# lizaibeim/mmla-audio

Measured on AMD Instinct MI355X. Metric: audio clips/sec (MFCC→logits) at 1/2/4/8 MI355X; MFCC max-abs-err vs librosa, higher is better.
Workload: dtype f16x3+f32

## Files before the change

### mmla_audio_amd/csrc/context.cpp

```cpp
#include <algorithm>
#include <cstdarg>
#include <cstdio>
#include <cstdlib>

#include "internal.h"

using namespace mmla;

namespace mmla __attribute__((visibility("hidden"))) {

int fail(mmla_ctx* c, int code, const char* fmt, ...) {
  char buf[512];
  va_list ap;
  va_start(ap, fmt);
  vsnprintf(buf, sizeof(buf), fmt, ap);
  va_end(ap);
  if (c) c->err = buf;
  return code;
}

static hipEvent_t prof_event(mmla_ctx* c) {
  if (!c->prof_pool.empty()) {
    hipEvent_t e = c->prof_pool.back();
    c->prof_pool.pop_back();
// ... 134 lines not shown
  double held = 0;
  for (size_t i = 0; i < c->ws_size.size(); ++i)
    if (!slot_kept((int)i)) held += (double)c->ws_size[i];
  int64_t fit = (int64_t)(((double)fr + held) * 0.9 / (od ? kOdBytesPerClip : kSiBytesPerClip));
  fit = fit / kMinMicrobatch * kMinMicrobatch;
  return std::max(kMinMicrobatch, std::min(cap, fit));
}

}

struct EnvSwitch {
  const char* name;
  bool mmla_ctx::*no;
  int mmla_ctx::*num;
};
static const EnvSwitch kEnvSwitches[] = {
    {"MMLA_DEBUG_FAIL_ALLOC", nullptr, &mmla_ctx::debug_fail_allocs},
    {"MMLA_NO_SIU", &mmla_ctx::siu, nullptr},
    {"MMLA_NO_SIPU", &mmla_ctx::sipu, nullptr},
    {"MMLA_NO_SIFIN", &mmla_ctx::sifin, nullptr},
    {"MMLA_NO_SIPAIR", &mmla_ctx::sipair, nullptr},
    {"MMLA_NO_SICHAIN", &mmla_ctx::sichain, nullptr},
    {"MMLA_NO_LSTM_SPLIT", &mmla_ctx::lstm_split, nullptr},
    {"MMLA_LSTM_SPLIT_MAX", nullptr, &mmla_ctx::lstm_split_max},
    {"MMLA_DEBUG_LSTM_SPIN", nullptr, &mmla_ctx::lstm_spin},
    {"MMLA_DEBUG_TRACE_GUARD", nullptr, &mmla_ctx::debug_trace_guard},
    {"MMLA_NO_SIPAD", &mmla_ctx::si_pad_feat, nullptr},
    {"MMLA_NO_ODU", &mmla_ctx::odu, nullptr},
    {"MMLA_NO_ODW", &mmla_ctx::odw, nullptr},
    {"MMLA_NO_VADW", &mmla_ctx::vadw, nullptr},
    {"MMLA_VADW", nullptr, &mmla_ctx::vadw_all},
    {"MMLA_RB_TILE", &mmla_ctx::rbs, nullptr},
    {"MMLA_NO_RBS_W1L", &mmla_ctx::rbs_w1l, nullptr},
    {"MMLA_NO_RBS_TAILPAIR", &mmla_ctx::rbs_tailpair, nullptr},
    {"MMLA_NO_PIN_OUT", &mmla_ctx::pin_small, nullptr},
};

extern "C" {

int mmla_abi_version(void) { return MMLA_ABI_VERSION; }

int mmla_create(int device, mmla_ctx** out) {
  if (!out) return MMLA_E_INVALID;
  *out = nullptr;
  int ndev = 0;
  if (hipGetDeviceCount(&ndev) != hipSuccess || ndev == 0) return MMLA_E_HIP;
  if (device < 0 || device >= ndev) return MMLA_E_INVALID;
  if (hipSetDevice(device) != hipSuccess) return MMLA_E_HIP;
  mmla_ctx* c = new mmla_ctx();
  c->device = device;
  for (const EnvSwitch& s : kEnvSwitches)
    if (const char* v = std::getenv(s.name)) {
      if (s.no) c->*s.no = std::atoi(v) == 0;
      else c->*s.num = std::atoi(v);
    }
  if (hipStreamCreateWithFlags(&c->own_stream, hipStreamDefault) != hipSuccess) {
    delete c;
    return MMLA_E_HIP;
  }
  c->stream = c->own_stream;
  if (hipMalloc(&c->range_dev, RW_COUNT * sizeof(int)) != hipSuccess ||
      hipMemset(c->range_dev, 0, RW_COUNT * sizeof(int)) != hipSuccess ||
      hipHostMalloc(&c->range_host, 2 * sizeof(int), hipHostMallocDefault) != hipSuccess) {
    mmla_destroy(c);
    return MMLA_E_HIP;
  }
// ... 173 lines not shown
```

### mmla_audio_amd/csrc/internal.h

```cpp
#pragma once
#include <hip/hip_runtime.h>

#include <cstdint>
#include <cstring>
#include <string>
#include <vector>

#include "../../include/mmla.h"
#include "nr.h"
#include "od_fe.h"
#include "mix.h"
#include "si_fe.h"
#include "ssim.h"
#include "vad.h"

namespace mmla __attribute__((visibility("hidden"))) {

constexpr int OD_H = 128, OD_W = 151, OD_PIX = OD_H * OD_W;
constexpr int OD_IMG = OD_PIX * 3;
constexpr int SI_T = 256, SI_D = 39;
constexpr int SI_NEED_SAMPLES = 160 * 259 + 400;
constexpr int CH[9] = {32, 32, 32, 64, 64, 64, 128, 128, 128};
constexpr bool POOL[9] = {true, false, false, true, false, false, true, false, false};

// ... 66 lines not shown
  double prof_work[MMLA_NSTAGES] = {0};
  int64_t prof_n[MMLA_NSTAGES] = {0};
  int device = 0;
  hipStream_t stream = nullptr;
  hipStream_t own_stream = nullptr;
  std::string err;
  OdFeTables* od_tables = nullptr;
  SiFeTables* si_tables = nullptr;
  bool od_loaded = false, si_loaded = false;
  mmla::OdNet od;
  mmla::SiNet si;
  std::vector<void*> od_allocs, si_allocs;
  std::vector<void*> si_head_allocs;
  std::vector<void*> ws;
  std::vector<size_t> ws_size;
  std::vector<size_t> ws_guard;
  int64_t od_mb = 0, si_mb = 0;
  int64_t od_mb_cap = mmla::kOdMicrobatch, si_mb_cap = mmla::kSiMicrobatch;
  int debug_fail_allocs = 0;
  int debug_trace_guard = 0;
  int precision = MMLA_PREC_F16X3;
  bool siu = true;
  bool sipu = true;
  bool sifin = true;
  bool sipair = true;
  bool sichain = true;
  bool si_pad_feat = true;
  bool odu = true;
  bool odw = true;
  bool vadw = true;
  int vadw_all = 0;
  bool rbs = true;
  bool rbs_w1l = true;
  bool rbs_tailpair = true;
  bool lstm_split = true;
  int lstm_split_max = 128;
  int lstm_spin = 0;
  int* range_dev = nullptr;
  int* range_host = nullptr;
  bool pin_small = true;
  int* range_map = nullptr;
  int* range_map_dev = nullptr;
  char* pin_out = nullptr;
  char* pin_out_dev = nullptr;
  char* pin_in = nullptr;
  int64_t lstm_split_reruns = 0;
  int64_t range_reruns = 0;
  bool od_f32_only = false, si_f32_only = false;
  bool si_base_f16_bad = false;
  VadState* vad_state = nullptr;
  int64_t vad_streams = 0;
  int32_t* cap_state = nullptr;
  int cap_cur = 0;
  int64_t cap_streams = 0;
  int32_t cap_rate = 0, cap_channels = 0, cap_channel = 0, cap_ir = 0, cap_or = 0;
  NrTables* nr_tables = nullptr;
  float* nr_thresh = nullptr;
  int64_t nr_profiles = 0;
  bool nr_ready = false;
  int32_t nr_bank_sr = 0;
  double ns_time_constant_s = 2.0, ns_thresh_n_mult = 2.0, ns_sigmoid_slope = 10.0;
  int32_t ns_sr = 16000;
};

namespace mmla __attribute__((visibility("hidden"))) {

// ... 128 lines not shown
```

### mmla_audio_amd/csrc/net_runners.cpp

```cpp
#include <algorithm>

#include "conv.h"
#include "conv_h3.h"
#include "internal.h"
#include "nets.h"
#include "odu.h"
#include "resblk.h"
#include "siu.h"

using namespace mmla;

namespace {

ConvArgs conv_args(const ConvW& w, const float* x, float* y, int n, int h, int wd, int stride,
                   const BnW* bn, int pro, int epi, const float* res) {
  ConvArgs a{};
  a.x = x;
  a.wt = w.wt;
  a.bias = w.bias;
  a.scale = bn ? bn->scale : nullptr;
  a.shift = bn ? bn->shift : nullptr;
  a.res = res;
  a.y = y;
  a.n = n;
// ... 93 lines not shown
}

double lstm_flops(int64_t n, int T, int D) { return 2.0 * n * T * 2 * (256.0 + D) * 1024.0; }

hipError_t lstm_run(mmla_ctx* c, const Arith& ar, const LstmW& L, const float* seq, int64_t n, int T, float* out) {
  if (ar.h3() && L.wth[0] && ar.split &&
      n <= std::min(c->lstm_split_max, bilstm_h3_split_max_clips())) {
    void* ws = nullptr;
    if (ws_get(c, S_LSTM, bilstm_h3_split_ws_bytes(), &ws) != MMLA_OK) return hipErrorOutOfMemory;
    return bilstm_h3_split_launch(seq, (int)n, T, 128, L.wth[0], L.wtl[0], L.wth[1], L.wtl[1],
                                  L.bias[0], L.bias[1], out, ar.range, L.ws[0], L.ws[1], ws,
                                  ar.timeout, c->lstm_spin, c->stream);
  }
  if (ar.h3() && L.wth[0])
    return bilstm_h3_launch(seq, (int)n, T, 128, L.wth[0], L.wtl[0], L.wth[1], L.wtl[1], L.bias[0],
                            L.bias[1], out, ar.range, L.ws[0], L.ws[1], c->stream);
  return bilstm_launch(seq, (int)n, T, 128, L.wcat[0], L.wcat[1], L.bias[0], L.bias[1], out,
                       c->stream);
}


enum OdPath {
  OD_STRIPS,
  OD_TILES,
  OD_ODU,
  OD_PAIR
};
struct OdChoice {
  OdPath path;
  bool stem;
  int strips;
  bool w1_lds;
  bool tail_pair;
};

bool strips_ok(const ResUnitW& B, bool pool, int h, int w) {
  return B.ca.wh && B.cb.wh && (!pool || B.sc.wh) && B.ca.cin_pad == B.ca.cin && B.ca.cout_pad == 32 &&
         B.cb.cin_pad == 32 && B.cb.cout_pad == 32 && B.cb.kh == 4 && B.cb.kw == 1 &&
         (!pool || (B.sc.cin_pad == B.ca.cin && B.sc.cout_pad == 32)) &&
         rbs_supported(h, w, B.ca.cin, B.ca.cout, pool);
}

bool tiles_ok(const ResUnitW& B, bool pool) {
  return B.ca.fh && B.cb.fh && B.cb.kpad == 4 * B.cb.cin && (!pool || B.sc.fh) &&
         resblk_supported(B.ca.cin, B.ca.cout, pool);
}

bool odu_ok(const ResUnitW& B, bool pool, int h, int w) {
  return B.ca.wh && B.cb.wh && (!pool || B.sc.wh) && odu_supported(h, w, B.ca.cin, B.ca.cout, pool) &&
         B.ca.cin_pad == B.ca.cin && B.ca.cout_pad == B.ca.cout && B.cb.cin == B.ca.cout &&
         B.cb.cout == B.ca.cout && B.cb.cin_pad == B.cb.cin && B.cb.cout_pad == B.cb.cout &&
         B.cb.kh == 4 && B.cb.kw == 1 &&
         (!pool || (B.sc.cin == B.ca.cin && B.sc.cout == B.ca.cout && B.sc.cout_pad == B.sc.cout));
}

OdChoice od_choose(const mmla_ctx* c, const Arith& ar, const ResUnitW& B, int b, int h, int w, int stop) {
  OdChoice k{OD_PAIR, false, 1, false, false};
  if (!ar.h3()) return k;
  if (c->rbs && strips_ok(B, POOL[b], h, w)) {
    k.path = OD_STRIPS;
    k.w1_lds = c->rbs_w1l && !POOL[b];
    k.tail_pair = c->rbs_tailpair && POOL[b];
  } else if (tiles_ok(B, POOL[b])) {
    k.path = OD_TILES;
  } else if (c->odu && odu_ok(B, POOL[b], h, w)) {
    k.path = OD_ODU;
    k.strips = c->odw && odu_two_strips(h, w, B.ca.cin, B.ca.cout, POOL[b]) ? 2 : 1;
  }
  k.stem = b == 0 && stop != 0 && (k.path == OD_STRIPS || k.path == OD_TILES);
  return k;
}

ResBlkArgs resblk_args(const ResUnitW& B, bool pool, bool fused, const float* x, float* y, int64_t n,
                       int h, int w, int* range_flag, const ConvW* stem, const uint8_t* img_u8,
                       const float* img_f32) {
  ResBlkArgs r{};
  r.x = x;
  r.y = y;
  r.w1h = fused ? B.ca.fh : B.ca.wh;
  r.w1l = fused ? B.ca.fl : B.ca.wl;
  r.b1 = B.ca.bias;
  r.u1 = B.ca.unscale();
  r.s1 = B.bn_in.scale;
  r.t1 = B.bn_in.shift;
  r.w2h = fused ? B.cb.fh : B.cb.wh;
  r.w2l = fused ? B.cb.fl : B.cb.wl;
  r.b2 = B.cb.bias;
  r.u2 = B.cb.unscale();
  r.s2 = B.bn_mid.scale;
  r.t2 = B.bn_mid.shift;
  if (pool) {
    r.wsh = fused ? B.sc.fh : B.sc.wh;
    r.wsl = fused ? B.sc.fl : B.sc.wl;
    r.bs = B.sc.bias;
    r.us = B.sc.unscale();
// ... 80 lines not shown
  const size_t big = (size_t)n * OD_PIX * 32;
  float *X, *T1, *T2, *SEQ, *H;
  CHK(ws_floats(c, S_X, big, &X));
  CHK(ws_floats(c, S_T1, big, &T1));
  CHK(ws_floats(c, S_T2, big, &T2));
  CHK(ws_floats(c, S_SEQ, (size_t)n * 19 * 128, &SEQ));
  CHK(ws_floats(c, S_HOUT, (size_t)n * 512, &H));
  const double stem_flops = 2.0 * n * OD_PIX * 3 * 16;
  const OdChoice first = od_choose(c, ar, W.blk[0], 0, OD_H, OD_W, stop);
  if (!first.stem)
    LAUNCH(c, MMLA_STAGE_GLUE, stem_flops,
           od_stem_launch(img_u8, img_f32, n * OD_PIX, W.stem.cout_pad, W.stem.wt, W.stem.bias, X,
                          c->stream));
  int h = OD_H, w = OD_W;
  if (stop == 0) {
    *tap = X;
    *tap_n = n * OD_PIX * 16;
    return MMLA_OK;
  }
  for (int b = 0; b < 9; ++b) {
    const ResUnitW& B = W.blk[b];
    const bool pool = POOL[b];
    const OdChoice k = b == 0 ? first : od_choose(c, ar, B, b, h, w, stop);
    const double flops = od_block_flops(B, pool, n, h, w) + (k.stem ? stem_flops : 0.0);
    float* out = T1;
    switch (k.path) {
      case OD_STRIPS:
      case OD_TILES: {
        const bool tiles = k.path == OD_TILES;
        const ResBlkArgs r = resblk_args(B, pool, tiles, X, T1, n, h, w, ar.range,
                                         k.stem ? &W.stem : nullptr, img_u8, img_f32);
        LAUNCH(c, MMLA_STAGE_CONV, flops,
               tiles ? resblk_launch(r, B.ca.cin, B.ca.cout, pool, c->stream)
                     : rbs_launch(r, B.ca.cin, B.ca.cout, pool, k.w1_lds, k.tail_pair, c->stream));
        break;
      }
      case OD_ODU: {
        const OduArgs o = odu_args(B, pool, X, T1, n, ar.range);
        LAUNCH(c, MMLA_STAGE_CONV, flops,
               odu_launch(o, h, w, B.ca.cin, B.ca.cout, pool, k.strips, c->stream));
        break;
      }
      case OD_PAIR:
        CHK(od_block_pair(c, ar, B, pool, (int)n, h, w, X, T1, T2, &out));
        break;
    }
    if (pool) {
      h = (h + 1) / 2;
      w = (w + 1) / 2;
    }
    if (out != X) std::swap(X, T1);
    if (stop == b + 1) {
      *tap = X;
      *tap_n = n * h * w * CH[b];
      return MMLA_OK;
    }
  }
  LAUNCH(c, MMLA_STAGE_GLUE, (double)n * h * w * 128,
         mean_h_launch(X, (int)n, h, w, 128, SEQ, c->stream));
  if (stop == 10) {
    *tap = SEQ;
    *tap_n = n * w * 128;
    return MMLA_OK;
  }
  LAUNCH(c, MMLA_STAGE_LSTM, lstm_flops(n, w, 128),
         lstm_run(c, ar, W.lstm, SEQ, n, w, H));
  if (stop == 11) {
// ... 179 lines not shown
```

### mmla_audio_amd/csrc/rbs.hip

```cpp
#define RBS_KERNEL rbs_kernel
#define RBS_W1L false
#include "rbs_body.h"

namespace {

template <int H, int W, int CIN, bool POOL, bool STEM>
hipError_t launch(const ResBlkArgs& a, hipStream_t s) {
  using G = SG<H, W, CIN, POOL>;
  const int64_t blocks = (int64_t)a.n * G::STRIPS;
  if (blocks > 0x7fffffffLL) return hipErrorInvalidValue;
  hipLaunchKernelGGL((rbs_kernel<H, W, CIN, POOL, STEM>), dim3((unsigned)blocks), dim3(NT), 0, s, a);
  return hipGetLastError();
}

}

#if RBS_TRACE
extern "C" int mmla_debug_rbs_trace(unsigned long long* out) {
  return hipMemcpyFromSymbol(out, HIP_SYMBOL(rbs_trace_buf), sizeof(rbs_trace_buf)) == hipSuccess ? 0 : -2;
}
#endif

bool rbs_supported(int h, int w, int cin, int c, bool pool) {
  return c == 32 && ((h == 128 && w == 151 && cin == 16 && pool) || (h == 64 && w == 76 && cin == 32 && !pool));
}

hipError_t rbs_launch(const ResBlkArgs& a, int cin, int c, bool pool, bool w1_lds, bool tail_pair, hipStream_t s) {
  if (a.n == 0) return hipSuccess;
  if (!rbs_supported(a.h, a.w, cin, c, pool) || !a.y || !a.w1h || !a.w1l || !a.w2h || !a.w2l)
    return hipErrorInvalidValue;
  if (pool) {
    if (!a.wsh || !a.wsl || !a.bs) return hipErrorInvalidValue;
    if (a.img8 || a.imgf) return tail_pair ? rbs_tp_launch(a, s) : launch<128, 151, 16, true, true>(a, s);
    return hipErrorInvalidValue;
  }
  if (!a.x || a.x == a.y) return hipErrorInvalidValue;
  return w1_lds ? rbs_w1l_launch(a, s) : launch<64, 76, 32, false, false>(a, s);
}
```

### mmla_audio_amd/csrc/rbs_body.h

```cpp
#pragma once
#include "f16x3.h"
#include "resblk.h"
#if !defined(RBS_KERNEL) || !defined(RBS_W1L)
#error "define RBS_KERNEL and RBS_W1L before including rbs_body.h"
#endif
#ifndef RBS_TAILPAIR
#define RBS_TAILPAIR false
#endif
#ifndef RBS_SC_DEDUP
#define RBS_SC_DEDUP false
#endif

namespace {

constexpr int NT = 256;
constexpr int TW = 16;
constexpr int R = 8;
constexpr int C = 32;
#ifndef RBS_TRACE
#define RBS_TRACE 0
#endif
#if RBS_TRACE
__device__ unsigned long long rbs_trace_buf[2048 * 4 * 4 * 8];
#define RBS_T(i) do { if (bid < 2048 && k >= 2 && k < 6) tt[i] = __builtin_amdgcn_s_memtime(); } while (0)
#define RBS_TFLUSH() do { if (bid < 2048 && k >= 2 && k < 6 && lane == 0) { for (int i_ = 0; i_ < 8; ++i_) rbs_trace_buf[(((size_t)bid * 4 + wave) * 4 + (k - 2)) * 8 + i_] = tt[i_]; } } while (0)
#else
#define RBS_T(i) do { } while (0)
#define RBS_TFLUSH() do { } while (0)
#endif

template <int H, int W, int CIN, bool POOL>
struct SG {
  static constexpr int XW = TW + 2;
  static constexpr int XRING = R + 2, TRING = R + 3;
  static constexpr int XROW = XW * CIN;
  static constexpr int XPLANE = XRING * XROW;
  static constexpr int TROW = TW * C;
  static constexpr int TPLANE = TRING * TROW;
  static constexpr int NCHUNK = H / R;
  static constexpr int STRIPS = (W + TW - 1) / TW;
  static constexpr int QPP = CIN / 4;
  static constexpr int MAXT = (R * XW * QPP + NT - 1) / NT;
  static constexpr int MAXT0 = (4 * XW * QPP + NT - 1) / NT;
  static constexpr int KPT = CIN / 16;
  static constexpr int KS1 = 9 * KPT, KS2 = 8;
  static constexpr bool W2L = CIN == 16;
  static constexpr int MINB = CIN == 16 ? 3 : 2;
  static constexpr int PF = 3;
  static constexpr int PD = CIN == 16 ? 1 : 2;
  static_assert(H % R == 0, "geometry");
  static_assert(NT % QPP == 0, "a thread's channel quad is fixed");
  static_assert(XROW <= 1024 && W * CIN * 4 < 65536 && W * 12 < 65536, "staging task fields");
};

template <int CIN>
MMLA_DEV int xoff(int slot, int x, int g) {
  constexpr int XROW = (TW + 2) * CIN;
  const int f = CIN == 32 ? ((x >> 1) & 3) : ((x >> 1) & 1);
  return slot * XROW + x * CIN + 8 * (g ^ f);
}
template <bool POOL>
// ... 6 lines not shown
__global__ void __launch_bounds__(NT, (SG<H, W, CIN, POOL>::MINB)) RBS_KERNEL(ResBlkArgs a) {
  using G = SG<H, W, CIN, POOL>;
  constexpr bool W1L = RBS_W1L;
  static_assert(!STEM || (CIN == 16 && POOL), "the stem feeds block 1");
  static_assert(POOL || CIN == C, "residual blocks keep their width");
  static_assert(!W1L || G::MINB == 2, "LDS-resident GEMM 1 weights: two workgroups per CU");
  constexpr int KS1L = W1L ? G::KS1 - 1 : 0;
  static_assert(!W1L || 4 * (G::XPLANE + G::TPLANE + KS1L * 512) + 3 * C * 4 <= 160 * 1024 / 2, "LDS of two workgroups");
  __shared__ __attribute__((aligned(16))) _Float16 sx[2 * G::XPLANE];
  __shared__ __attribute__((aligned(16))) _Float16 st[2 * G::TPLANE];
  __shared__ float4 spar[3 * C / 4 + (STEM ? 16 : 0)];
  __shared__ __attribute__((aligned(16))) _Float16 sw2[G::W2L ? 2 * G::KS2 * 512 : 8];
  __shared__ __attribute__((aligned(16))) _Float16 sw1[W1L ? 2 * KS1L * 512 : 8];

  const int tid = threadIdx.x, lane = tid & 63;
  const int wave = __builtin_amdgcn_readfirstlane(tid >> 6);
  const int h = lane >> 5;
  const uint32_t bid = xcd_block_id();
  constexpr bool TP = RBS_TAILPAIR, SCD = RBS_SC_DEDUP;
  static_assert(!TP || (STEM && W % TW == TW / 2 - 1), "paired tails: block 1, two 7-column tails in one strip");
  static_assert(!SCD || TP, "the de-duplicated shortcut stem belongs to the paired-tails kernel");
  constexpr int FS = TP ? G::STRIPS - 1 : G::STRIPS;
  const bool pair = TP && bid >= (uint32_t)a.n * FS;
  const int clip = pair ? 2 * (int)(bid - (uint32_t)a.n * FS) : (int)(bid / FS);
  const int w0 = pair ? FS * TW : (int)(bid - (uint32_t)clip * FS) * TW;
  const bool has_b = pair && clip + 1 < a.n;
  auto ring_col = [&](int x, int& part, int& iw) -> bool {
    part = TP && pair && x >= G::XW / 2;
    iw = w0 - 1 + x - (TP ? part * (G::XW / 2) : 0);
    return iw >= 0 && iw < W && (!TP || !part || has_b);
  };
  const int lofs = lane * 8;
  float rmax = 0.0f;

  float* const sp = reinterpret_cast<float*>(spar);
  if (tid < C) {
    const float s2 = a.s2[tid];
    sp[tid] = 16.0f * (s2 * a.u1);
    sp[C + tid] = 16.0f * fmaf(a.b1[tid], s2, a.t2[tid]);
    sp[2 * C + tid] = a.b2[tid];
  }
  if constexpr (STEM) {
    if (tid < 64) {
      const int co = tid >> 2, k = tid & 3;
      sp[3 * C + tid] = k < 3 ? a.wst[k * a.ldst + co] : a.bst[co];
    }
  }
  const __amdgpu_buffer_rsrc_t rw1h = w_rsrc(a.w1h), rw1l = w_rsrc(a.w1l);
  f16x8 w2h[G::W2L ? 1 : G::KS2], w2l[G::W2L ? 1 : G::KS2];
  if constexpr (G::W2L) {
    for (int e = tid; e < 2 * G::KS2 * 64; e += NT) {
      const int pl = e / (G::KS2 * 64), i = e - pl * (G::KS2 * 64);
      *reinterpret_cast<f16x8*>(sw2 + 8 * e) = *reinterpret_cast<const f16x8*>((pl ? a.w2l : a.w2h) + 8 * i);
    }
  } else {
    const __amdgpu_buffer_rsrc_t rw2h = w_rsrc(a.w2h), rw2l = w_rsrc(a.w2l);
#pragma unroll
    for (int s = 0; s < G::KS2; ++s) {
      w2h[s] = w_frag(rw2h, s * 512, lofs);
      w2l[s] = w_frag(rw2l, s * 512, lofs);
    }
  }
  f16x8 w1th[W1L ? G::KS1 - KS1L : 1], w1tl[W1L ? G::KS1 - KS1L : 1];
  if constexpr (W1L) {
    for (int e = tid; e < 2 * KS1L * 64; e += NT) {
      const int pl = e / (KS1L * 64), i = e - pl * (KS1L * 64);
      *reinterpret_cast<f16x8*>(sw1 + 8 * e) = *reinterpret_cast<const f16x8*>((pl ? a.w1l : a.w1h) + 8 * i);
    }
#pragma unroll
    for (int s = KS1L; s < G::KS1; ++s) {
      w1th[s - KS1L] = w_frag(rw1h, s * 512, lofs);
      w1tl[s - KS1L] = w_frag(rw1l, s * 512, lofs);
    }
  }
  f16x8 wsh_, wsl_;
  if constexpr (POOL) {
    wsh_ = w_frag(w_rsrc(a.wsh), 0, lofs);
    wsl_ = w_frag(w_rsrc(a.wsl), 0, lofs);
  }
  const int q = tid % G::QPP;
  float bnw[4][4];
  __syncthreads();
#pragma unroll
  for (int c = 0; c < 4; ++c) {
    const float s16 = 16.0f * a.s1[4 * q + c], t16 = 16.0f * a.t1[4 * q + c];
    if constexpr (STEM) {
      const float4 v = spar[3 * C / 4 + 4 * q + c];
      bnw[c][0] = s16 * v.x;
      bnw[c][1] = s16 * v.y;
      bnw[c][2] = s16 * v.z;
      bnw[c][3] = fmaf(s16, v.w, t16);
    } else {
      bnw[c][0] = s16;
      bnw[c][1] = t16;
    }
  }

  constexpr uint32_t ROWB = STEM ? 0u : (uint32_t)W * CIN * 4;
  const __amdgpu_buffer_rsrc_t rx = STEM ? w_rsrc(nullptr) :
      __builtin_amdgcn_make_buffer_rsrc(const_cast<float*>(a.x) + (int64_t)clip * H * W * CIN, (short)0,
                                        (int)(H * ROWB), 0x00020000);
  const bool im8 = STEM && a.img8 != nullptr;
  const __amdgpu_buffer_rsrc_t rimg = !STEM ? w_rsrc(nullptr) :
      __builtin_amdgcn_make_buffer_rsrc(im8 ? (void*)(a.img8 + (int64_t)clip * H * W * 3)
                                            : (void*)(a.imgf + (int64_t)clip * H * W * 3),
                                        (short)0, TP ? __builtin_amdgcn_readfirstlane((int)(H * W * 3 * (im8 ? 1 : 4)) * (has_b ? 2 : 1))
                                                     : (int)(H * W * 3 * (im8 ? 1 : 4)), 0x00020000);
  uint32_t tinfo[G::MAXT];
  uint32_t tsrc[TP ? G::MAXT : 1];
#pragma unroll
  for (int j = 0; j < G::MAXT; ++j) {
    const int t = tid + j * NT;
    const int px = t / G::QPP;
    const int rr = px / G::XW, x = px - rr * G::XW;
    int part, iw;
    const bool col_ok = ring_col(x, part, iw);
    const uint32_t tc = !col_ok ? 0u : STEM ? (uint32_t)iw * (a.img8 ? 3u : 12u) : (uint32_t)(iw * CIN + 4 * q) * 4u;
// ... 16 lines not shown
      return make_float4(__builtin_bit_cast(float, __builtin_amdgcn_raw_buffer_load_b32(rimg, off, 0, 0)),
                         __builtin_bit_cast(float, __builtin_amdgcn_raw_buffer_load_b32(rimg, off + 4u, 0, 0)),
                         __builtin_bit_cast(float, __builtin_amdgcn_raw_buffer_load_b32(rimg, off + 8u, 0, 0)), 0.f);
    } else {
      const uint32_t off = col_ok ? (uint32_t)ih * ROWB + (uint32_t)(iw * CIN + 4 * q) * 4u : 0x80000000u;
      return __builtin_bit_cast(float4, __builtin_amdgcn_raw_buffer_load_b128(rx, off, 0, 0));
    }
  };
  auto img_px = [&](float4 v) -> float4 {
    if (im8)
      return make_float4((float)__builtin_bit_cast(uint32_t, v.x), (float)__builtin_bit_cast(uint32_t, v.y),
                         (float)__builtin_bit_cast(uint32_t, v.z), 0.f);
    return v;
  };
  auto load_task = [&](int r0, int j) -> float4 {
    const uint32_t ti = tinfo[j];
    const uint32_t off = (ti >> 14) & 1u ? (uint32_t)((r0 + (int)((ti >> 10) & 15)) * (STEM ? W * 3 * (im8 ? 1 : 4) : (int)ROWB)) +
                                               (TP ? tsrc[TP ? j : 0] : ti >> 16)
                                         : 0x80000000u;
    if constexpr (STEM) {
      if (im8) {
        const uint32_t r = __builtin_amdgcn_raw_buffer_load_b8(rimg, off, 0, 0);
        const uint32_t g = __builtin_amdgcn_raw_buffer_load_b8(rimg, off + 1u, 0, 0);
        const uint32_t b = __builtin_amdgcn_raw_buffer_load_b8(rimg, off + 2u, 0, 0);
        return make_float4(__builtin_bit_cast(float, r), __builtin_bit_cast(float, g), __builtin_bit_cast(float, b), 0.f);
      }
      return make_float4(__builtin_bit_cast(float, __builtin_amdgcn_raw_buffer_load_b32(rimg, off, 0, 0)),
                         __builtin_bit_cast(float, __builtin_amdgcn_raw_buffer_load_b32(rimg, off + 4u, 0, 0)),
                         __builtin_bit_cast(float, __builtin_amdgcn_raw_buffer_load_b32(rimg, off + 8u, 0, 0)), 0.f);
    } else {
      return __builtin_bit_cast(float4, __builtin_amdgcn_raw_buffer_load_b128(rx, off, 0, 0));
    }
  };
  auto stage4 = [&](int o, bool in, float4 v, auto MASK_) {
    constexpr bool MASK = decltype(MASK_)::value;
    if constexpr (STEM) {
      if (!im8 && (!MASK || in) && nonfinite3(v.x, v.y, v.z)) rmax = SPLIT_MAX;
      v = img_px(v);
    }
    float u[4];
#pragma unroll
    for (int c = 0; c < 4; ++c) {
      if constexpr (STEM) {
        float acc = v.x * bnw[c][0];
        acc = fmaf(v.y, bnw[c][1], acc);
        acc = fmaf(v.z, bnw[c][2], acc);
        u[c] = acc + bnw[c][3];
      } else {
        u[c] = fmaf((&v.x)[c], bnw[c][0], bnw[c][1]);
      }
    }
    float e[4];
#pragma unroll
    for (int c = 0; c < 4; ++c) e[c] = (!MASK || in) ? elu16(u[c]) : 0.0f;
    rmax = fmaxf(rmax, amax4(e[0], e[1], e[2], e[3]));
    f16x4 hv, lv;
    split4(e[0], e[1], e[2], e[3], hv, lv);
    *reinterpret_cast<f16x4*>(sx + o) = hv;
    *reinterpret_cast<f16x4*>(sx + G::XPLANE + o) = lv;
  };
  auto stage_task = [&](int r0, int j, float4 v, auto MASK_) {
    const uint32_t ti = tinfo[j];
    if (((ti >> 14) & 3u) != 3u) return;
    const int rr = (int)((ti >> 10) & 15);
    uint32_t slot = (uint32_t)((r0 + 1) % G::XRING) + (uint32_t)rr;
    slot = min(slot, slot - (uint32_t)G::XRING);
    stage4((int)slot * G::XROW + (int)(ti & 1023), r0 + rr < H, v, MASK_);
  };
  for (int e = tid; e < 2 * G::XRING * G::XW * G::QPP; e += NT) {
    const int pl = e / (G::XRING * G::XW * G::QPP), r = e - pl * (G::XRING * G::XW * G::QPP);
    const int slot = r / (G::XW * G::QPP), x = (r / G::QPP) % G::XW, qq = r % G::QPP;
    int part, iw;
    if (!ring_col(x, part, iw))
      *reinterpret_cast<f16x4*>(sx + pl * G::XPLANE + xoff<CIN>(slot, x, qq >> 1) + 4 * (qq & 1)) = f16x4{};
  }
  const int n = lane & 31, nr = n >> 4, nc = n & 15;
  auto tile_ring = [&](int c, int dx) -> int {
    if (!(TP && pair)) return c + dx;
    const int p = c >= TW / 2, cl = c - p * (TW / 2);
    return p * (G::XW / 2) + (cl == TW / 2 - 1 ? G::XW / 2 - 1 : cl + dx);
  };
  int xco[3][G::KPT];
#pragma unroll
  for (int dx = 0; dx < 3; ++dx)
#pragma unroll
    for (int ks = 0; ks < G::KPT; ++ks) xco[dx][ks] = xoff<CIN>(0, tile_ring(nc, dx), G::KPT == 2 ? 2 * ks + h : h);

  f16x8 w1h[W1L ? 1 : G::PF], w1l[W1L ? 1 : G::PF];
  auto gemm1_issue = [&]() {
    if constexpr (!W1L) {
#pragma unroll
      for (int s = 0; s < G::PF; ++s) {
        w1h[s] = w_frag(rw1h, s * 512, lofs);
        w1l[s] = w_frag(rw1l, s * 512, lofs);
      }
    }
  };
  auto gemm1 = [&](int j0) -> f32x16 {
    f32x16 acc;
#pragma unroll
    for (int i = 0; i < 16; ++i) acc[i] = 0.0f;
    int xr[3];
// ... 44 lines not shown
    return acc;
  };
  auto t1_write = [&](int j0, const f32x16& acc) {
    const int j = j0 + nr;
    const uint32_t sl = (uint32_t)((j0 + 1) % G::TRING) + (uint32_t)nr;
    const int slot = (int)min(sl, sl - (uint32_t)G::TRING);
    if (j0 < H) {
#pragma unroll
      for (int jj = 0; jj < 4; ++jj) {
        const int c0 = 8 * jj + 4 * h;
        const float4 sv = spar[c0 / 4], cv = spar[C / 4 + c0 / 4];
        float e[4];
        e[0] = elu16(fmaf(acc[4 * jj + 0], sv.x, cv.x));
        e[1] = elu16(fmaf(acc[4 * jj + 1], sv.y, cv.y));
        e[2] = elu16(fmaf(acc[4 * jj + 2], sv.z, cv.z));
        e[3] = elu16(fmaf(acc[4 * jj + 3], sv.w, cv.w));
        rmax = fmaxf(rmax, amax4(e[0], e[1], e[2], e[3]));
        f16x4 hv, lv;
        split4(e[0], e[1], e[2], e[3], hv, lv);
        const int o = toff<POOL>(slot, j, nc, jj) + 4 * h;
        *reinterpret_cast<f16x4*>(st + o) = hv;
        *reinterpret_cast<f16x4*>(st + G::TPLANE + o) = lv;
      }
    } else {
#pragma unroll
      for (int jj = 0; jj < 4; ++jj) {
        const int o = toff<POOL>(slot, j, nc, jj) + 4 * h;
        *reinterpret_cast<f16x4*>(st + o) = f16x4{};
        *reinterpret_cast<f16x4*>(st + G::TPLANE + o) = f16x4{};
      }
    }
  };

  {
    constexpr int T0 = 4 * G::XW * G::QPP;
#pragma unroll
    for (int j = 0; j < G::MAXT0; ++j) {
      const int t = tid + j * NT;
      const int px = t / G::QPP;
      const int rr = px / G::XW, x = px - rr * G::XW;
      const int ih = rr - 1;
      int part, iw;
      const bool col_ok = ring_col(x, part, iw);
      const float4 v = load_src(ih, iw, col_ok, part);
      if (t < T0 && col_ok)
        stage4(xoff<CIN>((ih + 1) % G::XRING, x, q >> 1) + 4 * (q & 1), ih >= 0, v, std::true_type{});
    }
    for (int e = tid; e < 2 * G::TROW / 8; e += NT)
      *reinterpret_cast<f16x8*>(st + (e >= G::TROW / 8 ? G::TPLANE - G::TROW : 0) + 8 * e) = f16x8{};
  }
  __syncthreads();
  if (wave == 0) {
    gemm1_issue();
    const f32x16 acc = gemm1(0);
    t1_write(0, acc);
  }
  float4 preA[G::MAXT], preB[G::PD == 2 ? G::MAXT : 1];
#pragma unroll
  for (int j = 0; j < G::MAXT; ++j) preA[j] = load_task(3, j);
  if constexpr (G::PD == 2) {
#pragma unroll
    for (int j = 0; j < G::MAXT; ++j) preB[j] = load_task(3 + R, j);
  }
  __syncthreads();

  const int win = n >> 2;
  const int sc_part = TP && pair && win >= 4;
  const int sc_col = w0 + 2 * (win - 4 * sc_part);
  const bool sc_ok_tp = sc_col < W && (!sc_part || has_b);
  auto sc_ok = [&]() -> bool {
    if constexpr (TP) return sc_ok_tp; else return sc_col < W;
  };
  float bsc = 0.0f;
  if constexpr (POOL) bsc = a.bs[n];

#if RBS_TRACE
  unsigned long long tt[8];
#endif
  static_assert(G::NCHUNK % 2 == 0, "chunk pairs");
  auto chunk = [&](const int k, float4* pre) {
    RBS_T(0);
    const int rx0 = R * k + 3;
    const int j0 = R * k + 2 + 2 * wave;
    const int o0 = R * k + 2 * wave;
    if (k + 1 < G::NCHUNK) {
#pragma unroll
      for (int j = 0; j < G::MAXT; ++j) stage_task(rx0, j, pre[j], std::false_type{});
    } else {
#pragma unroll
      for (int j = 0; j < G::MAXT; ++j) stage_task(rx0, j, pre[j], std::true_type{});
    }
    gemm1_issue();
    RBS_T(1);
    __syncthreads();
    RBS_T(2);
    {
      const f32x16 acc = gemm1(j0);
// ... 147 lines not shown
      const int prow = (R / 2) * k + wave;
#pragma unroll
      for (int jj = 0; jj < 4; ++jj) {
        const int wdw = 2 * jj + h;
        const int op = TP && pair && jj >= 2;
        const int cc = w0 + 2 * (wdw - 4 * op);
        if (cc >= W || (TP && op && !has_b)) continue;
        float m0 = fmaf(acc[4 * jj + 0], a.u2, b2);
        float m1 = fmaf(acc[4 * jj + 1], a.u2, b2);
        float m2 = fmaf(acc[4 * jj + 2], a.u2, b2);
        float m3 = fmaf(acc[4 * jj + 3], a.u2, b2);
        if (cc + 1 >= W) {
          m1 = m0;
          m3 = m2;
        }
        const float mx = fmaxf(fmaxf(m0, m1), fmaxf(m2, m3)) + fmaf(sacc[4 * jj], a.us, bs);
        a.y[(((int64_t)(clip + op) * HP + prow) * WP + (w0 >> 1) + wdw - 4 * op) * C + co] = mx;
      }
    }
    RBS_T(7);
    RBS_TFLUSH();
  };
  if constexpr (G::PD == 2) {
#pragma unroll 1
    for (int k = 0; k < G::NCHUNK; k += 2) {
      chunk(k, preA);
      chunk(k + 1, preB);
    }
  } else {
#pragma unroll 1
    for (int k = 0; k < G::NCHUNK; ++k) chunk(k, preA);
  }
  if (!(rmax < SPLIT_MAX) && a.range_flag) *a.range_flag = 1;
}

}
```

### mmla_audio_amd/csrc/rbs_tp.hip

```cpp
#define RBS_KERNEL rbs_tp_kernel
#define RBS_W1L false
#define RBS_TAILPAIR true
#ifndef RBS_SC_DEDUP
#define RBS_SC_DEDUP true
#endif
#include "rbs_body.h"

#if RBS_TRACE
extern "C" int mmla_debug_rbs_tp_trace(unsigned long long* out) {
  return hipMemcpyFromSymbol(out, HIP_SYMBOL(rbs_trace_buf), sizeof(rbs_trace_buf)) == hipSuccess ? 0 : -2;
}
#endif

hipError_t rbs_tp_launch(const ResBlkArgs& a, hipStream_t s) {
  using G = SG<128, 151, 16, true>;
  const int64_t blocks = (int64_t)a.n * (G::STRIPS - 1) + (a.n + 1) / 2;
  if (blocks > 0x7fffffffLL) return hipErrorInvalidValue;
  hipLaunchKernelGGL((rbs_tp_kernel<128, 151, 16, true, true>), dim3((unsigned)blocks), dim3(NT), 0, s, a);
  return hipGetLastError();
}
```

### mmla_audio_amd/csrc/rbs_w1l.hip

```cpp
#define RBS_KERNEL rbs_w1l_kernel
#define RBS_W1L true
#include "rbs_body.h"

#if RBS_TRACE
extern "C" int mmla_debug_rbs_w1l_trace(unsigned long long* out) {
  return hipMemcpyFromSymbol(out, HIP_SYMBOL(rbs_trace_buf), sizeof(rbs_trace_buf)) == hipSuccess ? 0 : -2;
}
#endif

hipError_t rbs_w1l_launch(const ResBlkArgs& a, hipStream_t s) {
  using G = SG<64, 76, 32, false>;
  const int64_t blocks = (int64_t)a.n * G::STRIPS;
  if (blocks > 0x7fffffffLL) return hipErrorInvalidValue;
  hipLaunchKernelGGL((rbs_w1l_kernel<64, 76, 32, false, false>), dim3((unsigned)blocks), dim3(NT), 0, s, a);
  return hipGetLastError();
}
```

### mmla_audio_amd/csrc/resblk.h

```cpp
#pragma once
#include <hip/hip_runtime.h>
#include <stdint.h>

struct ResBlkArgs {
  const float* x;
  const uint16_t* w1h;
  const uint16_t* w1l;
  const float* b1;
  const float* s1;
  const float* t1;
  const uint16_t* w2h;
  const uint16_t* w2l;
  const float* b2;
  const float* s2;
  const float* t2;
  const uint16_t* wsh;
  const uint16_t* wsl;
  const float* bs;
  const uint8_t* img8;
  const float* imgf;
  const float* wst;
  const float* bst;
  int ldst;
  float* y;
  int n, h, w;
  int tiles_h, tiles_w;
  int* range_flag;
  float u1, u2, us;
};

int resblk_k1pad(int cin);
bool resblk_supported(int cin, int c, bool pool);
hipError_t resblk_launch(ResBlkArgs a, int cin, int c, bool pool, hipStream_t stream);
void resblk_split_weights(const float* w, int taps, int cin, int cout, int kpad, uint16_t* hi,
                          uint16_t* lo, bool frag, float wscale);

bool rbs_supported(int h, int w, int cin, int c, bool pool);
hipError_t rbs_launch(const ResBlkArgs& a, int cin, int c, bool pool, bool w1_lds, bool tail_pair,
                      hipStream_t stream);
hipError_t rbs_w1l_launch(const ResBlkArgs& a, hipStream_t stream);
hipError_t rbs_tp_launch(const ResBlkArgs& a, hipStream_t stream);
```

Baseline: 174,000.

## Add load-first prologue variant for W1L strip residual-block kernel

Adds an EARLY variant of the W1L strip kernel (non-pool blocks at 64x76). Its prologue issues the first input-row loads, the prefetch tasks, the BN parameters and all weight fragments into registers up front, then writes them to LDS, instead of staging weights through LDS with a barrier before touching the input. This lets global-load latency overlap and removes one __syncthreads. It also skips the ring zero-fill for interior strips. The cost is more register pressure from holding prefetched data and weight copies. Strip-level timing probes are added under the trace build flag, and the variant is on by default with an env switch to disable it.

New measurement: 174,100, median of 6. Within noise of the previous version (+0.1%).

```diff
diff --git a/mmla_audio_amd/csrc/context.cpp b/mmla_audio_amd/csrc/context.cpp
--- a/mmla_audio_amd/csrc/context.cpp
+++ b/mmla_audio_amd/csrc/context.cpp
@@ -190,6 +190,7 @@
     {"MMLA_VADW", nullptr, &mmla_ctx::vadw_all},
     {"MMLA_RB_TILE", &mmla_ctx::rbs, nullptr},
     {"MMLA_NO_RBS_W1L", &mmla_ctx::rbs_w1l, nullptr},
+    {"MMLA_NO_RBS_EARLY", &mmla_ctx::rbs_early, nullptr},
     {"MMLA_NO_RBS_TAILPAIR", &mmla_ctx::rbs_tailpair, nullptr},
     {"MMLA_NO_PIN_OUT", &mmla_ctx::pin_small, nullptr},
 };
diff --git a/mmla_audio_amd/csrc/internal.h b/mmla_audio_amd/csrc/internal.h
--- a/mmla_audio_amd/csrc/internal.h
+++ b/mmla_audio_amd/csrc/internal.h
@@ -122,6 +122,7 @@
   int vadw_all = 0;
   bool rbs = true;
   bool rbs_w1l = true;
+  bool rbs_early = true;
   bool rbs_tailpair = true;
   bool lstm_split = true;
   int lstm_split_max = 128;
diff --git a/mmla_audio_amd/csrc/net_runners.cpp b/mmla_audio_amd/csrc/net_runners.cpp
--- a/mmla_audio_amd/csrc/net_runners.cpp
+++ b/mmla_audio_amd/csrc/net_runners.cpp
@@ -149,6 +149,7 @@
   int strips;
   bool w1_lds;
   bool tail_pair;
+  bool early;
 };
 
 bool strips_ok(const ResUnitW& B, bool pool, int h, int w) {
@@ -172,12 +173,13 @@
 }
 
 OdChoice od_choose(const mmla_ctx* c, const Arith& ar, const ResUnitW& B, int b, int h, int w, int stop) {
-  OdChoice k{OD_PAIR, false, 1, false, false};
+  OdChoice k{OD_PAIR, false, 1, false, false, false};
   if (!ar.h3()) return k;
   if (c->rbs && strips_ok(B, POOL[b], h, w)) {
     k.path = OD_STRIPS;
     k.w1_lds = c->rbs_w1l && !POOL[b];
     k.tail_pair = c->rbs_tailpair && POOL[b];
+    k.early = c->rbs_early && k.w1_lds;
   } else if (tiles_ok(B, POOL[b])) {
     k.path = OD_TILES;
   } else if (c->odu && odu_ok(B, POOL[b], h, w)) {
@@ -324,7 +326,7 @@
                                          k.stem ? &W.stem : nullptr, img_u8, img_f32);
         LAUNCH(c, MMLA_STAGE_CONV, flops,
                tiles ? resblk_launch(r, B.ca.cin, B.ca.cout, pool, c->stream)
-                     : rbs_launch(r, B.ca.cin, B.ca.cout, pool, k.w1_lds, k.tail_pair, c->stream));
+                     : rbs_launch(r, B.ca.cin, B.ca.cout, pool, k.w1_lds, k.tail_pair, k.early, c->stream));
         break;
       }
       case OD_ODU: {
diff --git a/mmla_audio_amd/csrc/rbs.hip b/mmla_audio_amd/csrc/rbs.hip
--- a/mmla_audio_amd/csrc/rbs.hip
+++ b/mmla_audio_amd/csrc/rbs.hip
@@ -19,13 +19,17 @@
 extern "C" int mmla_debug_rbs_trace(unsigned long long* out) {
   return hipMemcpyFromSymbol(out, HIP_SYMBOL(rbs_trace_buf), sizeof(rbs_trace_buf)) == hipSuccess ? 0 : -2;
 }
+extern "C" int mmla_debug_rbs_strip_trace(unsigned long long* out) {
+  return hipMemcpyFromSymbol(out, HIP_SYMBOL(rbs_strip_buf), sizeof(rbs_strip_buf)) == hipSuccess ? 0 : -2;
+}
 #endif
 
 bool rbs_supported(int h, int w, int cin, int c, bool pool) {
   return c == 32 && ((h == 128 && w == 151 && cin == 16 && pool) || (h == 64 && w == 76 && cin == 32 && !pool));
 }
 
-hipError_t rbs_launch(const ResBlkArgs& a, int cin, int c, bool pool, bool w1_lds, bool tail_pair, hipStream_t s) {
+hipError_t rbs_launch(const ResBlkArgs& a, int cin, int c, bool pool, bool w1_lds, bool tail_pair, bool early,
+                      hipStream_t s) {
   if (a.n == 0) return hipSuccess;
   if (!rbs_supported(a.h, a.w, cin, c, pool) || !a.y || !a.w1h || !a.w1l || !a.w2h || !a.w2l)
     return hipErrorInvalidValue;
@@ -35,5 +39,6 @@
     return hipErrorInvalidValue;
   }
   if (!a.x || a.x == a.y) return hipErrorInvalidValue;
-  return w1_lds ? rbs_w1l_launch(a, s) : launch<64, 76, 32, false, false>(a, s);
+  if (w1_lds) return early ? rbs_w1e_launch(a, s) : rbs_w1l_launch(a, s);
+  return launch<64, 76, 32, false, false>(a, s);
 }
diff --git a/mmla_audio_amd/csrc/rbs_body.h b/mmla_audio_amd/csrc/rbs_body.h
--- a/mmla_audio_amd/csrc/rbs_body.h
+++ b/mmla_audio_amd/csrc/rbs_body.h
@@ -9,6 +9,9 @@
 #endif
 #ifndef RBS_SC_DEDUP
 #define RBS_SC_DEDUP false
+#endif
+#ifndef RBS_EARLY
+#define RBS_EARLY false
 #endif
 
 namespace {
@@ -21,12 +24,23 @@
 #define RBS_TRACE 0
 #endif
 #if RBS_TRACE
+#ifndef RBS_TRACE_STRIDE
+#define RBS_TRACE_STRIDE 1
+#endif
 __device__ unsigned long long rbs_trace_buf[2048 * 4 * 4 * 8];
-#define RBS_T(i) do { if (bid < 2048 && k >= 2 && k < 6) tt[i] = __builtin_amdgcn_s_memtime(); } while (0)
-#define RBS_TFLUSH() do { if (bid < 2048 && k >= 2 && k < 6 && lane == 0) { for (int i_ = 0; i_ < 8; ++i_) rbs_trace_buf[(((size_t)bid * 4 + wave) * 4 + (k - 2)) * 8 + i_] = tt[i_]; } } while (0)
+constexpr int RBS_NP = 10;
+__device__ unsigned long long rbs_strip_buf[2048 * 4 * RBS_NP];
+#define RBS_SAMPLED (bid % RBS_TRACE_STRIDE == 0 && bid / RBS_TRACE_STRIDE < 2048)
+#define RBS_P(i) do { if (RBS_SAMPLED) pp[i] = __builtin_amdgcn_s_memtime(); } while (0)
+#define RBS_PFLUSH() do { if (RBS_SAMPLED && lane == 0) { for (int i_ = 0; i_ < RBS_NP; ++i_) rbs_strip_buf[((size_t)(bid / RBS_TRACE_STRIDE) * 4 + wave) * RBS_NP + i_] = pp[i_]; } } while (0)
+#define RBS_T(i) do { if (RBS_SAMPLED && k >= 2 && k < 6) tt[i] = __builtin_amdgcn_s_memtime(); \
+                      if ((i) == 1 && k == 0) RBS_P(7); if ((i) == 7 && k == G::NCHUNK - 1) RBS_P(8); } while (0)
+#define RBS_TFLUSH() do { if (RBS_SAMPLED && k >= 2 && k < 6 && lane == 0) { for (int i_ = 0; i_ < 8; ++i_) rbs_trace_buf[(((size_t)(bid / RBS_TRACE_STRIDE) * 4 + wave) * 4 + (k - 2)) * 8 + i_] = tt[i_]; } } while (0)
 #else
 #define RBS_T(i) do { } while (0)
 #define RBS_TFLUSH() do { } while (0)
+#define RBS_P(i) do { } while (0)
+#define RBS_PFLUSH() do { } while (0)
 #endif
 
 template <int H, int W, int CIN, bool POOL>
@@ -99,9 +113,15 @@
   };
   const int lofs = lane * 8;
   float rmax = 0.0f;
+  constexpr bool EARLY = RBS_EARLY;
+  static_assert(!EARLY || (W1L && !STEM && !POOL && !TP), "the load-first strip start: blocks 2-3 with W1L");
+#if RBS_TRACE
+  unsigned long long pp[RBS_NP] = {};
+#endif
+  RBS_P(0);
 
   float* const sp = reinterpret_cast<float*>(spar);
-  if (tid < C) {
+  if (!EARLY && tid < C) {
     const float s2 = a.s2[tid];
     sp[tid] = 16.0f * (s2 * a.u1);
     sp[C + tid] = 16.0f * fmaf(a.b1[tid], s2, a.t2[tid]);
@@ -120,7 +140,7 @@
       const int pl = e / (G::KS2 * 64), i = e - pl * (G::KS2 * 64);
       *reinterpret_cast<f16x8*>(sw2 + 8 * e) = *reinterpret_cast<const f16x8*>((pl ? a.w2l : a.w2h) + 8 * i);
     }
-  } else {
+  } else if constexpr (!EARLY) {
     const __amdgpu_buffer_rsrc_t rw2h = w_rsrc(a.w2h), rw2l = w_rsrc(a.w2l);
 #pragma unroll
     for (int s = 0; s < G::KS2; ++s) {
@@ -129,7 +149,7 @@
     }
   }
   f16x8 w1th[W1L ? G::KS1 - KS1L : 1], w1tl[W1L ? G::KS1 - KS1L : 1];
-  if constexpr (W1L) {
+  if constexpr (W1L && !EARLY) {
     for (int e = tid; e < 2 * KS1L * 64; e += NT) {
       const int pl = e / (KS1L * 64), i = e - pl * (KS1L * 64);
       *reinterpret_cast<f16x8*>(sw1 + 8 * e) = *reinterpret_cast<const f16x8*>((pl ? a.w1l : a.w1h) + 8 * i);
@@ -147,9 +167,10 @@
   }
   const int q = tid % G::QPP;
   float bnw[4][4];
-  __syncthreads();
-#pragma unroll
-  for (int c = 0; c < 4; ++c) {
+  if constexpr (!EARLY) __syncthreads();
+  RBS_P(1);
+#pragma unroll
+  for (int c = 0; !EARLY && c < 4; ++c) {
     const float s16 = 16.0f * a.s1[4 * q + c], t16 = 16.0f * a.t1[4 * q + c];
     if constexpr (STEM) {
       const float4 v = spar[3 * C / 4 + 4 * q + c];
@@ -232,6 +253,60 @@
       return __builtin_bit_cast(float4, __builtin_amdgcn_raw_buffer_load_b128(rx, off, 0, 0));
     }
   };
+  float4 preA[G::MAXT], preB[G::PD == 2 ? G::MAXT : 1];
+  constexpr int NCP = (2 * KS1L * 64 + NT - 1) / NT;
+  float4 pv0[EARLY ? G::MAXT0 : 1];
+  float es1[4], et1[4], es2 = 0.f, eb1 = 0.f, et2 = 0.f, eb2 = 0.f;
+  f16x8 wcp[EARLY ? NCP : 1];
+  if constexpr (EARLY) {
+#pragma unroll
+    for (int j = 0; j < G::MAXT0; ++j) {
+      const int px = (tid + j * NT) / G::QPP;
+      const int rr = px / G::XW, x = px - rr * G::XW;
+      int part, iw;
+      const bool col_ok = ring_col(x, part, iw);
+      pv0[j] = load_src(rr - 1, iw, col_ok, part);
+    }
+    __builtin_amdgcn_sched_barrier(0);
+    RBS_P(2);
+#pragma unroll
+    for (int j = 0; j < G::MAXT; ++j) preA[j] = load_task(3, j);
+#pragma unroll
+    for (int j = 0; j < G::MAXT; ++j) preB[j] = load_task(3 + R, j);
+    __builtin_amdgcn_sched_barrier(0);
+    RBS_P(5);
+#pragma unroll
+    for (int c = 0; c < 4; ++c) {
+      es1[c] = a.s1[4 * q + c];
+      et1[c] = a.t1[4 * q + c];
+    }
+    es2 = a.s2[tid & (C - 1)];
+    eb1 = a.b1[tid & (C - 1)];
+    et2 = a.t2[tid & (C - 1)];
+    eb2 = a.b2[tid & (C - 1)];
+    __builtin_amdgcn_sched_barrier(0);
+    const __amdgpu_buffer_rsrc_t rw2h = w_rsrc(a.w2h), rw2l = w_rsrc(a.w2l);
+#pragma unroll
+    for (int s = 0; s < G::KS2; ++s) {
+      w2h[s] = w_frag(rw2h, s * 512, lofs);
+      w2l[s] = w_frag(rw2l, s * 512, lofs);
+    }
+#pragma unroll
+    for (int s = KS1L; s < G::KS1; ++s) {
+      w1th[s - KS1L] = w_frag(rw1h, s * 512, lofs);
+      w1tl[s - KS1L] = w_frag(rw1l, s * 512, lofs);
+    }
+    __builtin_amdgcn_sched_barrier(0);
+#pragma unroll
+    for (int j = 0; j < NCP; ++j) {
+      const int e0 = j * NT + wave * 64;
+      const bool lo = e0 >= KS1L * 64;
+      if ((j + 1) * NT <= 2 * KS1L * 64 || e0 < 2 * KS1L * 64)
+        wcp[j] = w_frag(lo ? rw1l : rw1h, (size_t)(e0 - (lo ? KS1L * 64 : 0)) * 8, lofs);
+    }
+    __builtin_amdgcn_sched_barrier(0);
+    RBS_P(1);
+  }
   auto stage4 = [&](int o, bool in, float4 v, auto MASK_) {
     constexpr bool MASK = decltype(MASK_)::value;
     if constexpr (STEM) {
@@ -267,7 +342,8 @@
     slot = min(slot, slot - (uint32_t)G::XRING);
     stage4((int)slot * G::XROW + (int)(ti & 1023), r0 + rr < H, v, MASK_);
   };
-  for (int e = tid; e < 2 * G::XRING * G::XW * G::QPP; e += NT) {
+  const bool ring_edge = EARLY ? w0 == 0 || w0 + TW >= W : true;
+  for (int e = tid; ring_edge && e < 2 * G::XRING * G::XW * G::QPP; e += NT) {
     const int pl = e / (G::XRING * G::XW * G::QPP), r = e - pl * (G::XRING * G::XW * G::QPP);
     const int slot = r / (G::XW * G::QPP), x = (r / G::QPP) % G::XW, qq = r % G::QPP;
     int part, iw;
@@ -378,8 +454,16 @@
     }
   };
 
+  if constexpr (!EARLY) RBS_P(2);
   {
     constexpr int T0 = 4 * G::XW * G::QPP;
+    if constexpr (EARLY) {
+#pragma unroll
+      for (int c = 0; c < 4; ++c) {
+        bnw[c][0] = 16.0f * es1[c];
+        bnw[c][1] = 16.0f * et1[c];
+      }
+    }
 #pragma unroll
     for (int j = 0; j < G::MAXT0; ++j) {
       const int t = tid + j * NT;
@@ -388,27 +472,44 @@
       const int ih = rr - 1;
       int part, iw;
       const bool col_ok = ring_col(x, part, iw);
-      const float4 v = load_src(ih, iw, col_ok, part);
+      float4 v;
+      if constexpr (EARLY) v = pv0[j]; else v = load_src(ih, iw, col_ok, part);
       if (t < T0 && col_ok)
         stage4(xoff<CIN>((ih + 1) % G::XRING, x, q >> 1) + 4 * (q & 1), ih >= 0, v, std::true_type{});
     }
     for (int e = tid; e < 2 * G::TROW / 8; e += NT)
       *reinterpret_cast<f16x8*>(st + (e >= G::TROW / 8 ? G::TPLANE - G::TROW : 0) + 8 * e) = f16x8{};
+    if constexpr (EARLY) {
+      if (tid < C) {
+        sp[tid] = 16.0f * (es2 * a.u1);
+        sp[C + tid] = 16.0f * fmaf(eb1, es2, et2);
+        sp[2 * C + tid] = eb2;
+      }
+#pragma unroll
+      for (int j = 0; j < NCP; ++j)
+        if ((j + 1) * NT <= 2 * KS1L * 64 || j * NT + wave * 64 < 2 * KS1L * 64)
+          *reinterpret_cast<f16x8*>(sw1 + 8 * (tid + j * NT)) = wcp[j];
+    }
   }
   __syncthreads();
+  RBS_P(3);
   if (wave == 0) {
     gemm1_issue();
     const f32x16 acc = gemm1(0);
     t1_write(0, acc);
   }
-  float4 preA[G::MAXT], preB[G::PD == 2 ? G::MAXT : 1];
-#pragma unroll
-  for (int j = 0; j < G::MAXT; ++j) preA[j] = load_task(3, j);
-  if constexpr (G::PD == 2) {
-#pragma unroll
-    for (int j = 0; j < G::MAXT; ++j) preB[j] = load_task(3 + R, j);
+  RBS_P(4);
+  if constexpr (!EARLY) {
+#pragma unroll
+    for (int j = 0; j < G::MAXT; ++j) preA[j] = load_task(3, j);
+    if constexpr (G::PD == 2) {
+#pragma unroll
+      for (int j = 0; j < G::MAXT; ++j) preB[j] = load_task(3 + R, j);
+    }
+    RBS_P(5);
   }
   __syncthreads();
+  RBS_P(6);
 
   const int win = n >> 2;
   const int sc_part = TP && pair && win >= 4;
@@ -622,6 +723,8 @@
     for (int k = 0; k < G::NCHUNK; ++k) chunk(k, preA);
   }
   if (!(rmax < SPLIT_MAX) && a.range_flag) *a.range_flag = 1;
+  RBS_P(9);
+  RBS_PFLUSH();
 }
 
 }
diff --git a/mmla_audio_amd/csrc/rbs_tp.hip b/mmla_audio_amd/csrc/rbs_tp.hip
--- a/mmla_audio_amd/csrc/rbs_tp.hip
+++ b/mmla_audio_amd/csrc/rbs_tp.hip
@@ -10,6 +10,9 @@
 extern "C" int mmla_debug_rbs_tp_trace(unsigned long long* out) {
   return hipMemcpyFromSymbol(out, HIP_SYMBOL(rbs_trace_buf), sizeof(rbs_trace_buf)) == hipSuccess ? 0 : -2;
 }
+extern "C" int mmla_debug_rbs_tp_strip_trace(unsigned long long* out) {
+  return hipMemcpyFromSymbol(out, HIP_SYMBOL(rbs_strip_buf), sizeof(rbs_strip_buf)) == hipSuccess ? 0 : -2;
+}
 #endif
 
 hipError_t rbs_tp_launch(const ResBlkArgs& a, hipStream_t s) {
diff --git a/mmla_audio_amd/csrc/rbs_w1e.hip b/mmla_audio_amd/csrc/rbs_w1e.hip
--- /dev/null
+++ b/mmla_audio_amd/csrc/rbs_w1e.hip
@@ -0,0 +1,21 @@
+#define RBS_KERNEL rbs_w1e_kernel
+#define RBS_W1L true
+#define RBS_EARLY true
+#include "rbs_body.h"
+
+#if RBS_TRACE
+extern "C" int mmla_debug_rbs_w1e_trace(unsigned long long* out) {
+  return hipMemcpyFromSymbol(out, HIP_SYMBOL(rbs_trace_buf), sizeof(rbs_trace_buf)) == hipSuccess ? 0 : -2;
+}
+extern "C" int mmla_debug_rbs_w1e_strip_trace(unsigned long long* out) {
+  return hipMemcpyFromSymbol(out, HIP_SYMBOL(rbs_strip_buf), sizeof(rbs_strip_buf)) == hipSuccess ? 0 : -2;
+}
+#endif
+
+hipError_t rbs_w1e_launch(const ResBlkArgs& a, hipStream_t s) {
+  using G = SG<64, 76, 32, false>;
+  const int64_t blocks = (int64_t)a.n * G::STRIPS;
+  if (blocks > 0x7fffffffLL) return hipErrorInvalidValue;
+  hipLaunchKernelGGL((rbs_w1e_kernel<64, 76, 32, false, false>), dim3((unsigned)blocks), dim3(NT), 0, s, a);
+  return hipGetLastError();
+}
diff --git a/mmla_audio_amd/csrc/rbs_w1l.hip b/mmla_audio_amd/csrc/rbs_w1l.hip
--- a/mmla_audio_amd/csrc/rbs_w1l.hip
+++ b/mmla_audio_amd/csrc/rbs_w1l.hip
@@ -5,6 +5,9 @@
 #if RBS_TRACE
 extern "C" int mmla_debug_rbs_w1l_trace(unsigned long long* out) {
   return hipMemcpyFromSymbol(out, HIP_SYMBOL(rbs_trace_buf), sizeof(rbs_trace_buf)) == hipSuccess ? 0 : -2;
+}
+extern "C" int mmla_debug_rbs_w1l_strip_trace(unsigned long long* out) {
+  return hipMemcpyFromSymbol(out, HIP_SYMBOL(rbs_strip_buf), sizeof(rbs_strip_buf)) == hipSuccess ? 0 : -2;
 }
 #endif
 
diff --git a/mmla_audio_amd/csrc/resblk.h b/mmla_audio_amd/csrc/resblk.h
--- a/mmla_audio_amd/csrc/resblk.h
+++ b/mmla_audio_amd/csrc/resblk.h
@@ -37,6 +37,7 @@
 
 bool rbs_supported(int h, int w, int cin, int c, bool pool);
 hipError_t rbs_launch(const ResBlkArgs& a, int cin, int c, bool pool, bool w1_lds, bool tail_pair,
-                      hipStream_t stream);
+                      bool early, hipStream_t stream);
 hipError_t rbs_w1l_launch(const ResBlkArgs& a, hipStream_t stream);
+hipError_t rbs_w1e_launch(const ResBlkArgs& a, hipStream_t stream);
 hipError_t rbs_tp_launch(const ResBlkArgs& a, hipStream_t stream);
```
